# tum-vision/tandem

Hardware: AMD Instinct MI355X
Metric: depth-maps/sec @ 640×480×7-view×3-stage; TSDF voxels integrated/sec (higher is better)
Workload: dtype f32; 1 GPU; 640x480 ref+6-src keyframe window, 3-stage cascade (48/32/8 hypotheses), view aggregation, fp32; independent windows, 4 in flight per GPU (one DrMvsnet engine each) x 1 GPU replica(s); trained weights recovered from the reference's exported tandem_512x320 model (same architecture), inputs resident in HBM; height=480, width=640, views=7, parallelism=replicas x1, 4 engines per GPU

## Files before the change

### tandem_amd/csrc/conv_march.h

```cpp
#pragma once
#include "march_plan.h"

namespace dr {

struct MarchArgs {
  const int *tap2d;
  MarchGeom geo;
  int NPO;
  int ncols, colsH, colsW;
  int R, PS;
  int NP;
  int nit;
  int wsec;
  int NU;
  int steps;
  int ncw;
  int i_sv, i_sz, i_sy, o_sv, o_sz, o_sy;
  int depth;
  int inHp;
  int rm;
  int wino;
  int *err;
};

// ... 267 lines not shown
      s += sg.zb - sg.za;
    }
  }
}

template <int NRP, int CT, int PT>
struct MarchWSet {
  float4 g[3][CT], d[4][PT];
};
template <int NRP, int CT, int PT>
__device__ inline void march_w_load(const float4 *tile, const float4 *wsec, const int (&sw)[NRP][4][PT], int r, MarchWSet<NRP, CT, PT> &o) {
#pragma unroll
  for (int k = 0; k < 3; ++k)
#pragma unroll
    for (int ct = 0; ct < CT; ++ct) o.g[k][ct] = wsec[((r * 3 + k) * CT + ct) * 64];
#pragma unroll
  for (int pt = 0; pt < PT; ++pt)
#pragma unroll
    for (int q = 0; q < 4; ++q) o.d[q][pt] = tile[sw[r][q][pt]];
}
template <int NRP, int CT, int PT>
__device__ inline void march_w_anchor(const MarchWSet<NRP, CT, PT> &o) {
#pragma unroll
  for (int k = 0; k < 3; ++k)
#pragma unroll
    for (int ct = 0; ct < CT; ++ct) asm volatile("" ::"v"(o.g[k][ct].x), "v"(o.g[k][ct].y), "v"(o.g[k][ct].z), "v"(o.g[k][ct].w));
#pragma unroll
  for (int q = 0; q < 4; ++q)
#pragma unroll
    for (int pt = 0; pt < PT; ++pt) asm volatile("" ::"v"(o.d[q][pt].x), "v"(o.d[q][pt].y), "v"(o.d[q][pt].z), "v"(o.d[q][pt].w));
}
DR_HD inline float march_w_u1(float g0, float g1h, float g2) { return fmaf(g0 + g2, 0.5f, g1h); }
DR_HD inline float march_w_u2(float g0, float g1h, float g2) { return fmaf(g0 + g2, 0.5f, -g1h); }
template <int NRP, int CT, int PT>
__device__ inline void march_w_compute(MarchWSet<NRP, CT, PT> &o, floatx4 (&acc)[4][CT][PT]) {
  float4 u[4][CT];
#pragma unroll
  for (int ct = 0; ct < CT; ++ct) {
    const float4 g0 = o.g[0][ct], gh = o.g[1][ct], g2 = o.g[2][ct];
    u[0][ct] = g0; u[3][ct] = g2;
#ifdef DR_WABL_NO_WT
    u[1][ct] = gh; u[2][ct] = gh;
#else
    u[1][ct] = make_float4(march_w_u1(g0.x, gh.x, g2.x), march_w_u1(g0.y, gh.y, g2.y), march_w_u1(g0.z, gh.z, g2.z), march_w_u1(g0.w, gh.w, g2.w));
    u[2][ct] = make_float4(march_w_u2(g0.x, gh.x, g2.x), march_w_u2(g0.y, gh.y, g2.y), march_w_u2(g0.z, gh.z, g2.z), march_w_u2(g0.w, gh.w, g2.w));
#endif
  }
#ifndef DR_WABL_NO_IT
  conv_w_transform<PT>(o.d);
#endif
  conv_w_mfma<CT, PT>(u, o.d, acc);
}

template <int CT, int PT>
__device__ inline void march_epilogue_w(const ConvArgs &a, const MarchArgs &m, floatx4 (&acc)[4][CT][PT], const float4 (&scv)[CT], const float4 (&biv)[CT], int raw,
                                        int wave, int j, int g, int ct0, int zc, int z, int py0, int px0) {
#pragma unroll
  for (int pt = 0; pt < PT; ++pt) {
    const int tau = wave * PT + pt;
    const int xt = tau % a.TXT, yt = tau / a.TXT;
    const int qy = py0 + yt, qx = px0 + xt * 16 + j;
    if (qy >= a.nPH || qx >= a.nPW) continue;
#pragma unroll
    for (int ct = 0; ct < CT; ++ct) {
      const int c0 = (ct0 + ct) * 16 + 4 * g;
      if (c0 >= a.rows_valid) continue;
      const floatx4 m0 = acc[0][ct][pt], m1 = acc[1][ct][pt], m2 = acc[2][ct][pt], m3 = acc[3][ct][pt];
      const floatx4 o[2] = {(m0 + m1) + m2, (m1 - m2) - m3};
      size_t obase[2];
      float4 ps[2], ad[2];
#pragma unroll
      for (int r = 0; r < 2; ++r) {
        const int oy = 2 * qy + r;
        obase[r] = march_out_index(a, m, zc, z, oy, qx, c0);
        ps[r] = ad[r] = make_float4(0.f, 0.f, 0.f, 0.f);
        if (raw == 2) ps[r] = *reinterpret_cast<const float4 *>(a.out + obase[r]);
        if (raw != 1 && a.add_mode) {
          size_t abase = obase[r];
          if (a.add_mode == 2) abase = (((size_t)(zc + z) * a.addH + (oy >> 1)) * a.addW + (qx >> 1)) * a.outC + c0;
          ad[r] = *reinterpret_cast<const float4 *>(a.add + abase);
// ... 61 lines not shown
        asm volatile("" ::: "memory");
        const bool last = z == sg.zb - 1;
        auto tile_of = [&](int i) {
          int sl = cur.slot0 + lo + i;
          sl = sl >= R ? sl - R : sl;
          return (const float4 *)(lds4 + (size_t)sl * m.PS);
        };
        auto wsec_of = [&](int i) { return wp + (size_t)(lo + i) * m.wsec; };
        MarchWSet<NRP, CT, PT> set[2];
        march_w_load<NRP, CT, PT>(tile_of(0), wsec_of(0), sw, 0, set[0]);
#pragma unroll
        for (int i = 0; i < 3; ++i) {
          if (i < nsec) {
#pragma unroll
            for (int r = 0; r < NRP; ++r) {
              const int t = i * NRP + r;
              if (r + 1 < NRP) march_w_load<NRP, CT, PT>(tile_of(i), wsec_of(i), sw, r + 1, set[(t + 1) & 1]);
              else if (i + 1 < nsec) march_w_load<NRP, CT, PT>(tile_of(i + 1), wsec_of(i + 1), sw, 0, set[(t + 1) & 1]);
              __builtin_amdgcn_sched_barrier(0);
              march_w_compute<NRP, CT, PT>(set[t & 1], acc);
              __builtin_amdgcn_sched_barrier(0);
              if (r + 1 < NRP || i + 1 < nsec) march_w_anchor<NRP, CT, PT>(set[(t + 1) & 1]);
              if (r == NRP - 1 && (lo + i == 0 || last)) {
                asm volatile("" ::: "memory");
                if (lane == 0) flags[kMarchReleased + wave] = idx0 + lo + i + 1;
              }
            }
          }
        }
        march_epilogue_w<CT, PT>(a, m, acc, scv, biv, raw, wave, j, g, ct0, zc, z, py0, px0);
        cur.next_step(m.geo, R);
      }
      L += sg.nl;
      s += sg.zb - sg.za;
    }
  }
}

template <int CI>
__device__ inline void march_producer(const ConvArgs &a, const MarchArgs &m, float4 *lds4, march_flag_t *flags, float4 *wl, int pw, int lane, int s0,
                                      int s1, int NUP, int CT) {
  const int ct0 = blockIdx.z * CT, NS = m.geo.KZ * m.geo.NPI;
  int rel[kMarchMaxIt];
  unsigned yx[kMarchMaxIt];
#pragma unroll
  for (int it = 0; it < kMarchMaxIt; ++it) march_piece_entry<CI>(a, m, pw, it, lane, rel[it], yx[it]);
  const int depth = m.depth;
  int L = 0;
  for (int po = 0; po < m.NPO; ++po) {
    if (po > 0 && !march_wait_released(flags, m.ncw, L, m.err, lane)) return;
    for (int e = pw; e < NS * NUP * CT; e += kMarchProducers)
      conv_a_dma16(a.wpk + march_weight_src(a, m, po, e, NUP, CT, ct0) + lane, march_uniform(conv_a_lds_addr(wl + (size_t)e * 64)));
    int flight = 0;
    for (int s = s0; s < s1;) {
      const MarchSeg sg = march_segment(m.geo, s, s1);
      int zc, py0, px0;
      march_tile_origin(a, m, sg.col, zc, py0, px0);
      const int iy0 = m.rm ? 0 : py0 * a.sy - a.py, ix0 = px0 * a.sx - a.px;
      for (int l = 0; l < sg.nl; ++l) {
        const int idx = L + l;
        int plane, pi;
        march_load_plane(m.geo, sg, l, plane, pi);
#ifndef DR_MABL_FREE
        if (idx >= m.R && march_released_now(flags, m.ncw) < idx - m.R + 1) {
          if (flight) {
            conv_a_wait_dma();
// ... 93 lines not shown
          for (int c = 0; c < FZ / 4; ++c) { xi[4 * c] = xv[k][c].x; xi[4 * c + 1] = xv[k][c].y; xi[4 * c + 2] = xv[k][c].z; xi[4 * c + 3] = xv[k][c].w; }
#pragma unroll
          for (int sft = 0; sft < 4; ++sft)
#pragma unroll
            for (int gq = 0; gq < FZ / 4; ++gq)
#pragma unroll
              for (int r = 0; r < 4; ++r) acc4[r] = __builtin_fmaf(wr[r][4 * gq + sft], xi[4 * gq + sft], acc4[r]);
          float4 o = make_float4(0.f, 0.f, 0.f, 0.f);
          if (in[k]) { o.x = (acc4[0] + fb.x) + up[k].x; o.y = (acc4[1] + fb.y) + up[k].y; o.z = (acc4[2] + fb.z) + up[k].z; o.w = (acc4[3] + fb.w) + up[k].w; }
          if (pos < m.NP) dst[conv_a_unit<16>(pos, cg)] = o;
        }
      }
      asm volatile("" ::: "memory");
      if (lane == 0) flags[pw] = idx + 1;
    }
    L += sg.nl;
    s += sg.zb - sg.za;
  }
}

template <int CI, int NUP, int CT, int PT, int FZ = 0, int NCW = 8, int W = 0>
__global__ __launch_bounds__(64 * (NCW + (FZ ? kMarchFzProducers : kMarchProducers))) void k_conv_m(const ConvArgs a, const MarchArgs m) {
  extern __shared__ float4 lds4[];
  const int tid = threadIdx.x, lane = tid & 63, wave = march_uniform(tid >> 6);
  float4 *wl = lds4 + (size_t)m.R * m.PS;
  march_flag_t *flags = (march_flag_t *)(__attribute__((address_space(3))) char *)(wl + (size_t)m.geo.KZ * m.geo.NPI * m.wsec);
  if (tid < kMarchFlagInts) flags[tid] = 0;
  __syncthreads();
  const int nwg = gridDim.x, id = (int)(blockIdx.x & 7u) * (nwg >> 3) + (int)(blockIdx.x >> 3);
  int s0, s1;
  march_range(m.steps, id, nwg, s0, s1);
  if (s0 >= s1) return;
  if (wave < NCW) {
    if constexpr (W) march_consumer_w<CI, NUP, CT, PT, kMarchProducers>(a, m, lds4, flags, wl, wave, lane, s0, s1);
    else march_consumer<CI, NUP, CT, PT, (FZ ? kMarchFzProducers : kMarchProducers)>(a, m, lds4, flags, wl, wave, lane, s0, s1);
  }
  else if constexpr (FZ > 0) march_producer_fz<FZ>(a, m, lds4, flags, wl, wave - NCW, lane, s0, s1, NUP, CT);
  else march_producer<CI>(a, m, lds4, flags, wl, wave - NCW, lane, s0, s1, NUP, CT);
}

}
```

### tandem_amd/csrc/conv_mfma.h

```cpp
#pragma once
#include <algorithm>
#include <atomic>
#include <functional>

#include "dr_common.h"

namespace dr {

typedef float floatx4 __attribute__((ext_vector_type(4)));

struct ConvClass {
  int NU;
  int tap_base;
  int w_base;
  int ooz, ooy, oox;
};

struct ConvArgs {
  const float *in;
  float *out;
  const float4 *wpk;
  const float *scale, *bias, *add;
  const int *tapoff;
  const ConvClass *cls;
// ... 800 lines not shown
      ptrs.push_back(d);
      return d;
    }
    T *d = dalloc<T>(h.size());
    DR_HIP(hipMemcpy(d, h.data(), h.size() * sizeof(T), hipMemcpyHostToDevice));
    ptrs.push_back(d);
    return d;
  }
  ~DeviceArena() { for (void *p : ptrs) { if (host_only) free(p); else dfree(p); } }
};

struct ConvTuned {
  int Cin, Cout, kd, kh, kw, sd, sh, sw, transposed, mode, inD, inH, inW;
  int ci, ct, pt, tz, ty, txt;
  int async_;
};
#include "conv_tuned.h"

inline bool conv_instance_exists(int ci, int ct) {
  return (ci == 4 && ct == 1) || ((ci == 8 || ci == 16) && (ct == 1 || ct == 2 || ct == 4));
}
inline bool conv_a_instance_exists(int ci, int ct, int pt) {
  return (pt == 1 || pt == 2 || pt == 4) && ((ci == 4 && ct == 1 && pt != 1) || ((ci == 8 || ci == 16) && (ct == 1 || ct == 2)));
}
#define DR_MARCH_INSTANCES(X)                                                                                         \
  X(8, 6, 1, 2, 8) X(8, 6, 1, 4, 8) X(8, 6, 1, 1, 12) X(8, 6, 1, 2, 12)                                               \
  X(16, 12, 1, 2, 8) X(16, 12, 1, 4, 8) X(16, 12, 1, 1, 12) X(16, 12, 1, 2, 12)                                       \
  X(16, 9, 1, 2, 8) X(16, 9, 1, 4, 8) X(16, 9, 1, 1, 12) X(16, 9, 1, 2, 12) X(16, 9, 2, 2, 8)                         \
  X(8, 2, 1, 1, 8) X(8, 2, 1, 2, 8) X(8, 2, 1, 4, 8) X(8, 2, 1, 1, 10) X(8, 2, 1, 2, 10)                              \
  X(16, 4, 1, 1, 8) X(16, 4, 1, 2, 8) X(16, 4, 1, 4, 8) X(16, 4, 1, 1, 10) X(16, 4, 1, 2, 10)                         \
  X(16, 3, 1, 1, 8) X(16, 3, 1, 2, 8) X(16, 3, 1, 4, 8) X(16, 3, 1, 1, 10) X(16, 3, 1, 2, 10)                         \
  X(16, 3, 2, 1, 8) X(16, 3, 2, 2, 8) X(16, 3, 2, 1, 10) X(16, 3, 2, 2, 10)
#define DR_MARCH_W_INSTANCES(X) X(8, 6, 1, 1, 8) X(16, 12, 1, 1, 8) X(16, 9, 1, 1, 8)
inline bool conv_m_instance_exists(int ci, int nup, int ct, int pt, int ncw, bool wino = false) {
#define DR_X(CI_, NUP_, CT_, PT_, NCW_) if (ci == CI_ && nup == NUP_ && ct == CT_ && pt == PT_ && ncw == NCW_) return true;
  if (wino) { DR_MARCH_W_INSTANCES(DR_X) return false; }
  DR_MARCH_INSTANCES(DR_X)
#undef DR_X
  return false;
}
inline int conv_march_policy() {
  if (const char *e = getenv("DR_CONV_MARCH")) return atoi(e);
  return 1;
}
inline int conv_rowmarch_policy() {
  if (const char *e = getenv("DR_CONV_ROWMARCH")) return atoi(e);
  return 1;
}
struct MarchShape {
  int nup, npi, npo, ns, tyi, txi, np, ps, r, ncw;
  size_t wbytes, lds_bytes;
  long long steps;
  int grid;
  bool ok;
};
inline MarchShape march_shape(int KZ, int ntp, int Cin, int ci, int ct, int pt, int ty, int txt, int SX, int exy, int exx, int nPD, int nPH, int nPW, int CTtot,
                              bool rm = false, bool wino = false) {
  MarchShape m{};
  const int tpc = 16 / ci;
  if (Cin % ci || ntp % tpc || CTtot % ct || (ty * txt) % pt || (rm && (ty != 1 || KZ != 1)) || (wino && (KZ != 3 || rm || (ntp / 3) % tpc))) return m;
  m.ncw = ty * txt / pt;
  m.nup = ntp / tpc;
  if (!conv_m_instance_exists(ci, m.nup, ct, pt, m.ncw, wino)) return m;
  const int npass = Cin / ci, kz = rm ? 3 : KZ;
  if (npass > 2) return m;
  m.npi = KZ == 1 ? npass : 1; m.npo = KZ == 1 ? 1 : npass; m.ns = kz * m.npi;
// ... 165 lines not shown
      if (in_split && ci != in_split) continue;
      if (ci == 8 && L.Cin != 8) continue;
      for (int ncw : {8, 12})
      for (int pt : {1, 2, 4})
        for (int ty = 1; ty <= ncw * pt; ++ty) {
          if ((ncw * pt) % ty) continue;
          const int txt = ncw * pt / ty;
          if ((ty > 1 && ty / 2 >= nPH) || (txt > 1 && (txt / 2) * 16 >= nPW)) continue;
          for (int ct : {2, 1}) {
            const MarchShape ms = march_shape(L.kd, march_ntp, L.Cin, ci, ct, pt, ty, txt, SX, exy, exx, nPD, nPH, nPW, CTtot);
            if (!ms.ok || (fz && (ci != 16 || ct != 1 || ncw != 8))) continue;
            const double spw = std::ceil((double)ms.steps / ms.grid);
            const double unit = ms.ns * ms.nup * 4.0 * ct * pt * 32.0 * (ncw / 4) * (ncw == 12 ? 0.94 : 1.0);
            const double startup = (double)ms.lds_bytes / 16.0 + 3000.0;
            double cost = ms.npo * (spw * unit * 1.02 + startup);
            if (fz) cost *= 1.5;
            else if (L.kd == 1) cost *= 1.6;
            if (march_policy >= 2) cost *= 1e-3;
            cands.push_back({cost, ci, pt, ct, 1, ty, txt, L.kd, ms.tyi, ms.txi, 2});
          }
        }
    }
  }
  const int wino_policy_m = (!fz && !bf3) ? conv_wino_policy() : 0;
  if (march_ok && wino_policy_m >= 1 && L.kd == 3 && (R.outH & 1) == 0 && R.outH >= 2) {
    const int nPHw = R.outH / 2;
    for (int ci : {16, 8}) {
      if (in_split && ci != in_split) continue;
      if (ci == 8 && L.Cin != 8) continue;
      for (int ncw : {8})
        for (int ty = 1; ty <= ncw; ++ty) {
          if (ncw % ty) continue;
          const int txt = ncw / ty;
          if ((ty > 1 && ty / 2 >= nPHw) || (txt > 1 && (txt / 2) * 16 >= nPW)) continue;
          const MarchShape ms = march_shape(L.kd, march_ntp, L.Cin, ci, 1, 1, ty, txt, SX, exy, exx, nPD, nPHw, nPW, CTtot, false, true);
          if (!ms.ok) continue;
          const double spw = std::ceil((double)ms.steps / ms.grid);
          const double unit = ms.ns * (ms.nup / 3) * 16.0 * 32.0 * (ncw / 4) * (ncw == 12 ? 0.94 : 1.0);
          const double startup = (double)ms.lds_bytes / 16.0 + 3000.0;
          double cost = ms.npo * (spw * unit * 1.1 + startup);
          if (wino_policy_m >= 2) cost *= 1e-3 * 0.5;
          cands.push_back({cost, ci, 1, 1, 1, ty, txt, L.kd, ms.tyi, ms.txi, 5});
        }
    }
  }
  const bool rowmarch_ok = !fz && !bf3 && conv_rowmarch_policy() >= 1 && ncls == 1 && !L.transposed && !L.up2 && mode != CONV_X8 && L.kd == 1 && L.kh == 3 && L.kw == 3 &&
                           SZ == 1 && SY == 1 && L.sw == 1 && !add;
  const int row_ntp = rowmarch_ok ? (int)cx[0].t.size() : 0;
  if (rowmarch_ok) {
    for (int ci : {16, 8}) {
      if (in_split && ci != in_split) continue;
      if (ci == 8 && L.Cin != 8) continue;
      for (int ncw : {8, 10})
        for (int pt : {1, 2, 4}) {
          const int txt = ncw * pt;
          if (txt > 1 && (txt / 2) * 16 >= nPW) continue;
          for (int ct : {2, 1}) {
            const MarchShape ms = march_shape(L.kd, row_ntp, L.Cin, ci, ct, pt, 1, txt, SX, exy, exx, nPD, nPH, nPW, CTtot, true);
            if (!ms.ok) continue;
            const double spw = std::ceil((double)ms.steps / ms.grid);
            const double waste = (double)cdiv(nPW, txt * 16) * txt * 16 / nPW;
            const double unit = ms.ns * ms.nup * 4.0 * ct * pt * 32.0 * (ncw / 4.0) + 300.0;
            const double startup = (double)ms.lds_bytes / 16.0 + 3000.0;
            double cost = (spw * unit * 1.02 + startup) * 1.5;
            (void)waste;
            if (conv_rowmarch_policy() >= 2) cost *= 1e-3;
            cands.push_back({cost, ci, pt, ct, 1, 1, txt, 1, 1, ms.txi, 3});
// ... 273 lines not shown
    }
    const int ntiles = a.tilesD * a.tilesH * a.tilesW, split = CTtot / CT;
    const int wpc = cl.lds_bytes * 2 <= kConvMaxLds ? 2 : 1;
    const int want = std::max(1, std::min(ntiles, 256 * wpc / split));
    cl.grid = dim3(8 * cdiv(want, 8), 1, split);
  }
  if (ASYNC == 2 || ASYNC == 3 || ASYNC == 5) {
    const bool rm = ASYNC == 3;
    const MarchShape ms = rm ? march_shape(L.kd, row_ntp, L.Cin, CI, CT, PT, 1, TXT, SX, exy, exx, nPD, nPH, nPW, CTtot, true)
                             : march_shape(L.kd, march_ntp, L.Cin, CI, CT, PT, TY, TXT, SX, exy, exx, nPD, nPH, nPW, CTtot, false, wino_raw);
    if (!ms.ok) fail(DR_ERR_ARG, "plan_conv: inconsistent k_conv_m plan");
    cl.async = 2; cl.nup = ms.nup; cl.ncw = ms.ncw;
    a.zero16 = arena.upload(std::vector<float>(4, 0.f));
    a.a_slots = 0; a.a_wbufs = 0;
    MarchArgs &m = cl.march;
    const int kz = rm ? 3 : L.kd;
    std::vector<int> tap2d((size_t)ms.nup * TPC, 0);
    {
      const DimTaps &Y = *classes[0].y, &X = *classes[0].x;
      int n = 0;
      if (rm) for (size_t ix = 0; ix < X.t.size(); ++ix, ++n) tap2d[n] = X.off[ix];
      else for (size_t iy = 0; iy < Y.t.size(); ++iy) for (size_t ix = 0; ix < X.t.size(); ++ix, ++n) tap2d[n] = Y.off[iy] * TXI + X.off[ix];
    }
    m.tap2d = arena.upload(tap2d);
    m.geo.KZ = kz; m.geo.NPI = ms.npi; m.geo.Dc = rm ? nPH : (L.kd == 3 ? nPD : 1);
    m.NPO = ms.npo;
    m.colsH = rm ? 1 : cdiv(nPH, TY); m.colsW = cdiv(nPW, TXT * 16);
    m.ncols = (L.kd == 3 ? 1 : nPD) * m.colsH * m.colsW;
    m.R = ms.r; m.PS = ms.ps; m.NP = ms.np; m.nit = ms.ps / 128;
    m.wsec = ms.nup * CT * 64; m.NU = kz * ms.nup;
    m.steps = (int)ms.steps;
    m.ncw = ms.ncw;
    m.rm = rm ? 1 : 0;
    m.wino = wino_raw ? 1 : 0;
    const long long iplane = (long long)a.inH * a.inW * a.inC, oplane = (long long)a.outH * a.outW * a.outC;
    if (iplane * std::max(1, a.inD) >= (1ll << 31) || oplane * std::max(1, a.outD) >= (1ll << 31)) fail(DR_ERR_ARG, "plan_conv: tensor too large for k_conv_m's 32-bit strides");
    m.i_sv = L.kd == 3 ? 0 : (int)iplane; m.i_sz = rm ? a.inW * a.inC : (L.kd == 3 ? (int)iplane : 0); m.i_sy = rm ? 0 : a.inW * a.inC;
    m.o_sv = L.kd == 3 ? 0 : (int)oplane; m.o_sz = rm ? a.outW * a.outC : (L.kd == 3 ? (int)oplane : 0); m.o_sy = rm ? 0 : a.outW * a.outC;
    m.inHp = rm ? 1 : a.inH;
    m.err = arena.err_flag;
    m.depth = rm ? 3 : 2;
    if (const char *e = hook_env("DR_MARCH_PDEPTH")) m.depth = std::max(1, std::min(4, atoi(e)));
    cl.lds_bytes = ms.lds_bytes;
    cl.grid = dim3(ms.grid, 1, CTtot / CT);
  }
  cl.flops = flops;
  R.launches.push_back(cl);
  return R;
}

inline void conv_allow_big_lds(const void *fn, std::atomic<unsigned long long> &done, size_t lds_bytes) {
  if (lds_bytes <= 64 * 1024) return;
  int dev = 0;
  DR_HIP(hipGetDevice(&dev));
  const unsigned long long bit = 1ull << (dev & 63);
  if (done.load(std::memory_order_acquire) & bit) return;
  DR_HIP(hipFuncSetAttribute(fn, hipFuncAttributeMaxDynamicSharedMemorySize, (int)kConvMaxLds));
  done.fetch_or(bit, std::memory_order_release);
}
template <int CI, int CT, int PT, int FZ = 0>
inline void launch_conv_inst(const ConvLaunch &c, hipStream_t st) {
  static std::atomic<unsigned long long> done{0};
  conv_allow_big_lds(reinterpret_cast<const void *>(&k_conv<CI, CT, PT, FZ>), done, c.lds_bytes);
  hipLaunchKernelGGL((k_conv<CI, CT, PT, FZ>), c.grid, dim3(kConvThreads), c.lds_bytes, st, c.args);
}
#ifdef DR_PARITY_HOOKS
template <int CI, int CT, int PT>
// ... 28 lines not shown
  hipLaunchKernelGGL((k_conv_m<CI, NUP, CT, PT, FZ, NCW, W>), c.grid, dim3(64 * (NCW + (FZ ? kMarchFzProducers : kMarchProducers))), c.lds_bytes, st, c.args, c.march);
}
inline void launch_conv(const ConvLaunch &c, hipStream_t st) {
#ifndef DR_PARITY_HOOKS
  if (c.bf3) fail(DR_ERR_UNSUPPORTED, "launch_conv: the bf16 x 3 kernel is built with -DDR_PARITY_HOOKS only");
#else
  if (c.bf3) {
#define DR_CONV_B_CASE(CI_, CT_)                                                \
  if (c.ci == CI_ && c.ct == CT_ && !c.async && !c.fz) {                        \
    if (c.pt == 4) launch_conv_b_inst<CI_, CT_, 4>(c, st);                      \
    else launch_conv_b_inst<CI_, CT_, 1>(c, st);                                \
    return;                                                                     \
  }
    DR_CONV_B_CASE(8, 1)
    DR_CONV_B_CASE(8, 2)
    DR_CONV_B_CASE(8, 4)
    DR_CONV_B_CASE(16, 1)
    DR_CONV_B_CASE(16, 2)
    DR_CONV_B_CASE(16, 4)
#undef DR_CONV_B_CASE
    fail(DR_ERR_ARG, "launch_conv: no bf16x3 instance CI=%d CT=%d", c.ci, c.ct);
  }
#endif
#ifndef DR_PARITY_HOOKS
  if (c.fz) fail(DR_ERR_UNSUPPORTED, "launch_conv: fused-skip kernels are built with -DDR_PARITY_HOOKS only");
#else
  if (c.async == 2 && c.fz) {
    if (c.fz != 8 || c.ci != 16 || c.nup != 12 || c.ct != 1 || c.ncw != 8) fail(DR_ERR_ARG, "launch_conv: no fused-skip marching instance FZ=%d CI=%d NUP=%d CT=%d", c.fz, c.ci, c.nup, c.ct);
    if (c.pt == 4) launch_conv_m_inst<16, 12, 1, 4, 8>(c, st);
    else launch_conv_m_inst<16, 12, 1, 2, 8>(c, st);
    return;
  }
#endif
  if (c.async == 2 && c.march.wino) {
#define DR_X(CI_, NUP_, CT_, PT_, NCW_) \
  if (c.ci == CI_ && c.nup == NUP_ && c.ct == CT_ && c.pt == PT_ && c.ncw == NCW_) { launch_conv_m_inst<CI_, NUP_, CT_, PT_, 0, NCW_, 1>(c, st); return; }
    DR_MARCH_W_INSTANCES(DR_X)
#undef DR_X
    fail(DR_ERR_ARG, "launch_conv: no Winograd marching instance CI=%d NUP=%d CT=%d PT=%d waves=%d", c.ci, c.nup, c.ct, c.pt, c.ncw);
  }
  if (c.async == 2) {
#define DR_X(CI_, NUP_, CT_, PT_, NCW_) \
  if (c.ci == CI_ && c.nup == NUP_ && c.ct == CT_ && c.pt == PT_ && c.ncw == NCW_) { launch_conv_m_inst<CI_, NUP_, CT_, PT_, 0, NCW_>(c, st); return; }
    DR_MARCH_INSTANCES(DR_X)
#undef DR_X
    fail(DR_ERR_ARG, "launch_conv: no marching instance CI=%d NUP=%d CT=%d PT=%d waves=%d", c.ci, c.nup, c.ct, c.pt, c.ncw);
  }
  if (c.async == 4) {
#define DR_CONV_W_CASE(CI_, CT_, PT_) if (c.ci == CI_ && c.ct == CT_ && c.pt == PT_) { launch_conv_w_inst<CI_, CT_, PT_>(c, st); return; }
    DR_CONV_W_CASE(16, 1, 1) DR_CONV_W_CASE(16, 1, 2) DR_CONV_W_CASE(16, 2, 1) DR_CONV_W_CASE(16, 2, 2)
    DR_CONV_W_CASE(8, 1, 1) DR_CONV_W_CASE(8, 1, 2)
#undef DR_CONV_W_CASE
    fail(DR_ERR_ARG, "launch_conv: no Winograd instance CI=%d CT=%d PT=%d", c.ci, c.ct, c.pt);
  }
  if (c.async) {
#define DR_CONV_A_CASE(CI_, CT_)                                                \
  if (c.ci == CI_ && c.ct == CT_) {                                             \
    if (c.pt == 4) launch_conv_a_inst<CI_, CT_, 4>(c, st);                      \
    else if (c.pt == 2) launch_conv_a_inst<CI_, CT_, 2>(c, st);                 \
    else launch_conv_a_inst<CI_, CT_, 1>(c, st);                                \
    return;                                                                     \
  }
    if (c.ci == 4 && c.ct == 1 && c.pt == 1) fail(DR_ERR_ARG, "launch_conv: no async instance CI=4 PT=1");
    DR_CONV_A_CASE(4, 1)
    DR_CONV_A_CASE(8, 1)
    DR_CONV_A_CASE(8, 2)
    DR_CONV_A_CASE(16, 1)
    DR_CONV_A_CASE(16, 2)
#undef DR_CONV_A_CASE
    fail(DR_ERR_ARG, "launch_conv: no async instance CI=%d CT=%d PT=%d", c.ci, c.ct, c.pt);
  }
// ... 41 lines not shown
```

### tandem_amd/csrc/dr_mvsnet.hip

```cpp
#include <atomic>
#include <memory>

#include <dlfcn.h>
#include <rccl/rccl.h>

#include "conv_mfma.h"
#include "mvs_host.h"
#include "mvs_launch.h"
#ifdef DR_PARITY_HOOKS
#include "tail_kernels.h"
#endif
#include "fn_front.h"
#include "fn_head3.h"

namespace dr {

std::string &last_error_slot() {
  thread_local std::string s;
  return s;
}

struct DevTensor {
  float *d = nullptr;
  int D = 0, H = 0, W = 0, C = 0;
// ... 1274 lines not shown
    L.transposed = transposed == 1; L.weight = weight; L.relu = relu != 0;
    const bool up2 = transposed == 2;
    if (scale) L.scale.assign(scale, scale + Cout);
    if (bias) L.bias.assign(bias, bias + Cout);
    const ConvMode mode = (!transposed && sw == 1 && Cout == 8) ? CONV_XPAIR : ((!transposed && sw == 1 && Cout == 1) ? CONV_X8 : CONV_NORMAL);
    auto cz = axis_classes(kd, sd, L.transposed, D), cy = axis_classes(kh, sh, L.transposed, H), cx = axis_classes(kw, sw, L.transposed, W);
    const int oD = L.transposed ? D * sd : cz[0].npos, oH = L.transposed ? H * sh : (up2 ? 2 * H : cy[0].npos), oW = L.transposed ? W * sw : (up2 ? 2 * W : cx[0].npos);
    std::vector<float> hin(in, in + (size_t)D * H * W * Cin);
    float *d_in = arena.upload(hin);
    const size_t on = (size_t)oD * oH * oW * Cout;
    float poison; memcpy(&poison, &guard::kWord, 4);
    float *d_out = arena.upload(std::vector<float>(on, poison));
    float *d_add = nullptr;
    if (add) {
      const size_t an = add_up2 ? (size_t)oD * (oH / 2) * (oW / 2) * Cout : on;
      std::vector<float> ha(add, add + an);
      d_add = arena.upload(ha);
    }
    const char *rk = getenv("DR_CONV_RANK");
    ConvPlanOut P;
    for (int py = 0; py < (up2 ? 2 : 1); ++py) {
      L.up2 = up2 ? 1 + py : 0;
      P = plan_conv(L, mode, d_in, D, H, W, Cin, d_out, d_add, add_up2 ? 2 : 1, arena, rk ? atoi(rk) : 0);
      for (auto &cl : P.launches) launch_conv(cl, nullptr);
    }
    DR_HIP(hipDeviceSynchronize());
    DR_HIP(hipGetLastError());
    int march_err = 0;
    DR_HIP(hipMemcpy(&march_err, arena.err_flag, sizeof(int), hipMemcpyDeviceToHost));
    if (march_err) fail(DR_ERR_DEVICE, "k_conv_m: a ring wait gave up (code %d)", march_err);
    if (getenv("DR_CONV_PRINT")) {
      const ConvLaunch &c = P.launches.at(0);
      fprintf(stderr, "debug_conv: %s<%d,%d,%d> nup %d tile %dx%dx%d lds %zu grid %ux%u (%d candidates)%s\n", *conv_kind_name(c) ? conv_kind_name(c) : (c.bf3 ? "bf16x3" : "sync"), c.ci, c.ct, c.pt,
              c.nup, c.args.TZ, c.args.TY, c.args.TXT * 16, c.lds_bytes, c.grid.x, c.grid.z, P.ncand, c.args.class_loop ? ", class loop" : "");
    }
    DR_HIP(hipMemcpy(out, d_out, on * 4, hipMemcpyDeviceToHost));
    if (out_dims) { out_dims[0] = oD; out_dims[1] = oH; out_dims[2] = oW; }
  });
}

int drm_debug_tail(int device, const float *x, const float *skip, const float *w_deconv, const float *scale8, const float *bias8, const float *w_prob, int D, int h,
                   int w, int qy, int zchunk, int form, float *out) {
  return guarded([&] {
    using namespace dr;
#ifndef DR_PARITY_HOOKS
    fail(DR_ERR_UNSUPPORTED, "drm_debug_tail: k_tail / k_tail_m are built into the parity library (libdr_mi355x_hooks.so, -DDR_PARITY_HOOKS) only");
#else
    int n = 0;
    if (hipGetDeviceCount(&n) != hipSuccess || n <= device) fail(DR_ERR_DEVICE, "no HIP device %d", device);
    if (D <= 0 || h <= 0 || w <= 0 || (D | h | w) & 1) fail(DR_ERR_ARG, "drm_debug_tail: output dims must be positive and even");
    DR_HIP(hipSetDevice(device));
    DeviceArena arena;
    TailArgs t{};
    t.x = arena.upload(std::vector<float>(x, x + (size_t)(D / 2) * (h / 2) * (w / 2) * 16));
    t.skip = arena.upload(std::vector<float>(skip, skip + (size_t)D * h * w * 8));
    t.wd = arena.upload(tail_pack_deconv(w_deconv));
    std::vector<float> sb(scale8, scale8 + 8);
    sb.insert(sb.end(), bias8, bias8 + 8);
    t.sb = arena.upload(sb);
    t.wp = arena.upload(tail_pack_prob(w_prob));
    float poison; memcpy(&poison, &guard::kWord, 4);
    float *d_out = arena.upload(std::vector<float>((size_t)D * h * w, poison));
    t.out = d_out; t.D = D; t.h = h; t.w = w;
    const bool mf = form == 1;
    t.wmf = mf ? arena.upload(tail_pack_deconv_mfma(w_deconv)) : nullptr;
    tail_set_tile(t, qy, zchunk, mf);
    launch_tail(t, nullptr);
// ... 9 lines not shown
```

### tandem_amd/csrc/march_plan.h

```cpp
#pragma once
#if defined(__HIPCC__)
#define DR_HD __host__ __device__
#else
#define DR_HD
#endif

namespace dr {

struct MarchGeom {
  int Dc;
  int KZ;
  int NPI;
};
struct MarchSeg {
  int col, za, zb;
  int p0;
  int nl;
};

DR_HD inline MarchSeg march_segment(const MarchGeom &g, int s, int s1) {
  MarchSeg r;
  r.col = s / g.Dc;
  r.za = s - r.col * g.Dc;
  r.zb = r.za + (s1 - s) < g.Dc ? r.za + (s1 - s) : g.Dc;
// ... 2 lines not shown
    const int p1 = r.zb < g.Dc ? r.zb : g.Dc - 1;
    r.nl = (p1 - r.p0 + 1) * g.NPI;
  } else {
    r.p0 = r.za;
    r.nl = (r.zb - r.za) * g.NPI;
  }
  return r;
}
DR_HD inline int march_section_load(const MarchGeom &g, const MarchSeg &sg, int z, int sec) {
  const int dz = sec / g.NPI, pi = sec - dz * g.NPI;
  const int plane = g.KZ == 3 ? z - 1 + dz : z;
  if (plane < 0 || plane >= g.Dc) return -1;
  return (plane - sg.p0) * g.NPI + pi;
}
DR_HD inline bool march_section_releases(const MarchGeom &g, const MarchSeg &sg, int z, int sec) {
  return g.KZ == 1 || sec / g.NPI == 0 || z == sg.zb - 1;
}
DR_HD inline void march_load_plane(const MarchGeom &g, const MarchSeg &sg, int l, int &plane, int &pi) {
  plane = sg.p0 + l / g.NPI;
  pi = l % g.NPI;
}
struct MarchCursor {
  int rel0, slot0;
  DR_HD void begin(const MarchGeom &g, const MarchSeg &sg, int L, int R) {
    rel0 = (sg.za - (g.KZ == 3 ? 1 : 0) - sg.p0) * g.NPI;
    slot0 = (L + rel0 + 2 * R) % R;
  }
  DR_HD void next_step(const MarchGeom &g, int R) {
    rel0 += g.NPI;
    slot0 = slot0 + g.NPI >= R ? slot0 + g.NPI - R : slot0 + g.NPI;
  }
};

DR_HD inline void march_range(long long steps, int id, int n, int &s0, int &s1) {
  s0 = (int)(steps * id / n);
  s1 = (int)(steps * (id + 1) / n);
}

}
```

Before: 591.2 depth-maps/s.

## Add scatter-order Winograd marching consumer that reuses each input plane across three outputs

Adds a new Winograd marching-conv consumer that visits each loaded input depth plane once and scatters its contribution into three rotating output accumulators (one per kernel z-tap), instead of gathering three planes per output step. Each input tile is read and input-transformed once per plane rather than once per kz tap. The aim is to cut LDS traffic and repeated input transforms. In exchange it triples the accumulator register footprint, which risks register pressure and lower occupancy. It also changes ring release timing and makes this path the default, keeping the old gather order only behind an env var in parity builds.

```diff
diff --git a/tandem_amd/csrc/conv_march.h b/tandem_amd/csrc/conv_march.h
--- a/tandem_amd/csrc/conv_march.h
+++ b/tandem_amd/csrc/conv_march.h
@@ -323,12 +323,11 @@
 }
 DR_HD inline float march_w_u1(float g0, float g1h, float g2) { return fmaf(g0 + g2, 0.5f, g1h); }
 DR_HD inline float march_w_u2(float g0, float g1h, float g2) { return fmaf(g0 + g2, 0.5f, -g1h); }
-template <int NRP, int CT, int PT>
-__device__ inline void march_w_compute(MarchWSet<NRP, CT, PT> &o, floatx4 (&acc)[4][CT][PT]) {
-  float4 u[4][CT];
+template <int CT>
+__device__ inline void march_w_derive(const float4 (&g)[3][CT], float4 (&u)[4][CT]) {
 #pragma unroll
   for (int ct = 0; ct < CT; ++ct) {
-    const float4 g0 = o.g[0][ct], gh = o.g[1][ct], g2 = o.g[2][ct];
+    const float4 g0 = g[0][ct], gh = g[1][ct], g2 = g[2][ct];
     u[0][ct] = g0; u[3][ct] = g2;
 #ifdef DR_WABL_NO_WT
     u[1][ct] = gh; u[2][ct] = gh;
@@ -337,6 +336,11 @@
     u[2][ct] = make_float4(march_w_u2(g0.x, gh.x, g2.x), march_w_u2(g0.y, gh.y, g2.y), march_w_u2(g0.z, gh.z, g2.z), march_w_u2(g0.w, gh.w, g2.w));
 #endif
   }
+}
+template <int NRP, int CT, int PT>
+__device__ inline void march_w_compute(MarchWSet<NRP, CT, PT> &o, floatx4 (&acc)[4][CT][PT]) {
+  float4 u[4][CT];
+  march_w_derive<CT>(o.g, u);
 #ifndef DR_WABL_NO_IT
   conv_w_transform<PT>(o.d);
 #endif
@@ -464,6 +468,175 @@
         cur.next_step(m.geo, R);
       }
       L += sg.nl;
+      s += sg.zb - sg.za;
+    }
+  }
+}
+
+template <int CT>
+struct MarchSG { float4 g[3][CT]; };
+template <int PT>
+struct MarchSD { float4 d[4][PT]; };
+template <int K>
+struct MarchPath { static constexpr int value = K; };
+template <int CT>
+__device__ inline void march_s_load_g(const float4 *wsec, int r, MarchSG<CT> &o) {
+#pragma unroll
+  for (int k = 0; k < 3; ++k)
+#pragma unroll
+    for (int ct = 0; ct < CT; ++ct) o.g[k][ct] = wsec[((r * 3 + k) * CT + ct) * 64];
+}
+template <int NRP, int PT>
+__device__ inline void march_s_load_d(const float4 *tile, const unsigned (&sw)[NRP][2][PT], int r, MarchSD<PT> &o) {
+  const char *tb = reinterpret_cast<const char *>(tile);
+#pragma unroll
+  for (int pt = 0; pt < PT; ++pt)
+#pragma unroll
+    for (int h = 0; h < 2; ++h) {
+      const unsigned x = sw[r][h][pt];
+      o.d[2 * h][pt] = *reinterpret_cast<const float4 *>(tb + (x & 0xffffu));
+      o.d[2 * h + 1][pt] = *reinterpret_cast<const float4 *>(tb + (x >> 16));
+    }
+}
+template <int CT>
+__device__ inline void march_s_anchor_g(const MarchSG<CT> &o) {
+#pragma unroll
+  for (int k = 0; k < 3; ++k)
+#pragma unroll
+    for (int ct = 0; ct < CT; ++ct) asm volatile("" ::"v"(o.g[k][ct].x), "v"(o.g[k][ct].y), "v"(o.g[k][ct].z), "v"(o.g[k][ct].w));
+}
+template <int PT>
+__device__ inline void march_s_anchor_d(const MarchSD<PT> &o) {
+#pragma unroll
+  for (int q = 0; q < 4; ++q)
+#pragma unroll
+    for (int pt = 0; pt < PT; ++pt) asm volatile("" ::"v"(o.d[q][pt].x), "v"(o.d[q][pt].y), "v"(o.d[q][pt].z), "v"(o.d[q][pt].w));
+}
+
+template <int CI, int NUP, int CT, int PT, int NPW>
+__device__ inline void march_consumer_ws(const ConvArgs &a, const MarchArgs &m, float4 *lds4, march_flag_t *flags, const float4 *wl, int wave, int lane,
+                                         int s0, int s1) {
+  static_assert(NUP % 3 == 0 && NUP >= 6, "three kernel rows per chunk of x taps, at least two chunks per plane");
+  constexpr int TPC = 16 / CI, NRP = NUP / 3, NG = 3 * NRP;
+  constexpr int WSEC = NUP * CT * 64;
+  const int j = lane & 15, g = lane >> 4;
+  const int sub = (4 * g) / CI, c4 = ((4 * g) % CI) / 4, ct0 = blockIdx.z * CT;
+  unsigned sw[NRP][2][PT];
+#pragma unroll
+  for (int pt = 0; pt < PT; ++pt) {
+    const int bpos = march_bpos(a, wave, pt, PT, j);
+#pragma unroll
+    for (int r = 0; r < NRP; ++r)
+#pragma unroll
+      for (int h = 0; h < 2; ++h) {
+        const unsigned lo = 16u * (unsigned)conv_a_unit<CI>(bpos + m.tap2d[r * TPC + sub] + (2 * h) * a.TXI, c4);
+        const unsigned hi = 16u * (unsigned)conv_a_unit<CI>(bpos + m.tap2d[r * TPC + sub] + (2 * h + 1) * a.TXI, c4);
+        sw[r][h][pt] = lo | (hi << 16);
+        asm volatile("" : "+v"(sw[r][h][pt]));
+      }
+  }
+  const float4 *wp = wl + lane;
+  const int R = m.R, Dc = m.geo.Dc;
+  floatx4 acc[3][4][CT][PT];
+  auto clear = [&](floatx4 (&s)[4][CT][PT]) {
+#pragma unroll
+    for (int p = 0; p < 4; ++p)
+#pragma unroll
+      for (int ct = 0; ct < CT; ++ct)
+#pragma unroll
+        for (int pt = 0; pt < PT; ++pt) s[p][ct][pt] = floatx4{0.f, 0.f, 0.f, 0.f};
+  };
+  auto move = [&](floatx4 (&d)[4][CT][PT], const floatx4 (&s)[4][CT][PT]) {
+#pragma unroll
+    for (int p = 0; p < 4; ++p)
+#pragma unroll
+      for (int ct = 0; ct < CT; ++ct)
+#pragma unroll
+        for (int pt = 0; pt < PT; ++pt) {
+          d[p][ct][pt] = s[p][ct][pt];
+        }
+  };
+  clear(acc[0]); clear(acc[1]); clear(acc[2]);
+  MarchSD<PT> dd[2];
+  MarchSG<CT> gg[2];
+  int cached = 0, idx = 0, slot = 0;
+  for (int po = 0; po < m.NPO; ++po) {
+    const int raw = m.NPO == 1 ? 0 : (po == 0 ? 1 : 2);
+    for (int s = s0; s < s1;) {
+      const MarchSeg sg = march_segment(m.geo, s, s1);
+      int zc, py0, px0;
+      march_tile_origin(a, m, sg.col, zc, py0, px0);
+      for (int i = 0; i < sg.nl; ++i) {
+        const int p = sg.p0 + i;
+        const bool more = i + 1 < sg.nl || s + (sg.zb - sg.za) < s1;
+        const bool on[3] = {march_plane_feeds(sg, p, 0), march_plane_feeds(sg, p, 1), march_plane_feeds(sg, p, 2)};
+        const float4 *tile = lds4 + (size_t)slot * m.PS;
+        auto plane = [&](auto main_path) -> bool {
+          constexpr bool MAIN = decltype(main_path)::value != 0;
+          if (!march_wait_ready<NPW>(flags, idx, cached, m.err, lane)) return false;
+          asm volatile("" ::: "memory");
+          march_s_load_g<CT>(wp, 0, gg[0]);
+          march_s_load_d<NRP, PT>(tile, sw, 0, dd[0]);
+#pragma unroll
+          for (int r = 0; r < NRP; ++r) {
+#pragma unroll
+            for (int dz = 0; dz < 3; ++dz) {
+              const int t = r * 3 + dz;
+              MarchSG<CT> &gn = gg[(t + 1) & 1];
+              MarchSD<PT> &dn = dd[(r + 1) & 1];
+              if (t + 1 < NG) {
+                march_s_load_g<CT>(wp + (size_t)((dz + 1) % 3) * WSEC, dz == 2 ? r + 1 : r, gn);
+                if (dz == 2) march_s_load_d<NRP, PT>(tile, sw, r + 1, dn);
+              }
+              __builtin_amdgcn_sched_barrier(0);
+              if (dz == 0) conv_w_transform<PT>(dd[r & 1].d);
+              if (MAIN || on[dz]) {
+                float4 u[4][CT];
+                march_w_derive<CT>(gg[t & 1].g, u);
+                conv_w_mfma<CT, PT>(u, dd[r & 1].d, acc[2 - dz]);
+              }
+              __builtin_amdgcn_sched_barrier(0);
+              if (t + 1 < NG) {
+                march_s_anchor_g<CT>(gn);
+                if (dz == 2) march_s_anchor_d<PT>(dn);
+              }
+              if ((MAIN || more) ? (r == NRP - 2 && dz == 2) : t == NG - 2) {
+                asm volatile("" ::: "memory");
+                if (lane == 0) flags[kMarchReleased + wave] = idx + 1;
+              }
+            }
+          }
+          const float *scp = a.scale, *bip = a.bias;
+          int el = lane;
+          asm volatile("" : "+s"(scp), "+s"(bip), "+v"(el));
+          const int j = el & 15, g = el >> 4;
+          float4 scv[CT], biv[CT];
+          if (MAIN || on[2] || on[1]) {
+#pragma unroll
+            for (int ct = 0; ct < CT; ++ct) {
+              scv[ct] = *reinterpret_cast<const float4 *>(scp + (ct0 + ct) * 16 + 4 * g);
+              biv[ct] = *reinterpret_cast<const float4 *>(bip + (ct0 + ct) * 16 + 4 * g);
+            }
+          }
+          if (MAIN || on[2]) {
+            march_epilogue_w<CT, PT>(a, m, acc[0], scv, biv, raw, wave, j, g, ct0, zc, p - 1, py0, px0);
+          }
+          if (!MAIN && on[1] && p == Dc - 1) {
+            march_epilogue_w<CT, PT>(a, m, acc[1], scv, biv, raw, wave, j, g, ct0, zc, p, py0, px0);
+            clear(acc[1]);
+          }
+          __builtin_amdgcn_sched_barrier(0);
+          move(acc[0], acc[1]);
+          move(acc[1], acc[2]);
+          clear(acc[2]);
+          __builtin_amdgcn_sched_barrier(0);
+          return true;
+        };
+        const bool inner = more && on[0] && on[1] && on[2];
+        if (!(inner ? plane(MarchPath<1>{}) : plane(MarchPath<0>{}))) return;
+        ++idx;
+        slot = slot + 1 == R ? 0 : slot + 1;
+      }
       s += sg.zb - sg.za;
     }
   }
@@ -623,7 +796,8 @@
   march_range(m.steps, id, nwg, s0, s1);
   if (s0 >= s1) return;
   if (wave < NCW) {
-    if constexpr (W) march_consumer_w<CI, NUP, CT, PT, kMarchProducers>(a, m, lds4, flags, wl, wave, lane, s0, s1);
+    if constexpr (W == 2) march_consumer_ws<CI, NUP, CT, PT, kMarchProducers>(a, m, lds4, flags, wl, wave, lane, s0, s1);
+    else if constexpr (W) march_consumer_w<CI, NUP, CT, PT, kMarchProducers>(a, m, lds4, flags, wl, wave, lane, s0, s1);
     else march_consumer<CI, NUP, CT, PT, (FZ ? kMarchFzProducers : kMarchProducers)>(a, m, lds4, flags, wl, wave, lane, s0, s1);
   }
   else if constexpr (FZ > 0) march_producer_fz<FZ>(a, m, lds4, flags, wl, wave - NCW, lane, s0, s1, NUP, CT);
diff --git a/tandem_amd/csrc/conv_mfma.h b/tandem_amd/csrc/conv_mfma.h
--- a/tandem_amd/csrc/conv_mfma.h
+++ b/tandem_amd/csrc/conv_mfma.h
@@ -856,6 +856,11 @@
   X(16, 3, 1, 1, 8) X(16, 3, 1, 2, 8) X(16, 3, 1, 4, 8) X(16, 3, 1, 1, 10) X(16, 3, 1, 2, 10)                         \
   X(16, 3, 2, 1, 8) X(16, 3, 2, 2, 8) X(16, 3, 2, 1, 10) X(16, 3, 2, 2, 10)
 #define DR_MARCH_W_INSTANCES(X) X(8, 6, 1, 1, 8) X(16, 12, 1, 1, 8) X(16, 9, 1, 1, 8)
+inline int conv_march_w_order(int ci, int nup) {
+  (void)ci; (void)nup;
+  if (const char *e = hook_env("DR_MARCH_W_ORDER")) return atoi(e) == 1 ? 1 : 2;
+  return 2;
+}
 inline bool conv_m_instance_exists(int ci, int nup, int ct, int pt, int ncw, bool wino = false) {
 #define DR_X(CI_, NUP_, CT_, PT_, NCW_) if (ci == CI_ && nup == NUP_ && ct == CT_ && pt == PT_ && ncw == NCW_) return true;
   if (wino) { DR_MARCH_W_INSTANCES(DR_X) return false; }
@@ -1087,7 +1092,7 @@
         for (int ty = 1; ty <= ncw; ++ty) {
           if (ncw % ty) continue;
           const int txt = ncw / ty;
-          if ((ty > 1 && ty / 2 >= nPHw) || (txt > 1 && (txt / 2) * 16 >= nPW)) continue;
+          if (!hook_env("DR_MARCH_ANY_TILE") && ((ty > 1 && ty / 2 >= nPHw) || (txt > 1 && (txt / 2) * 16 >= nPW))) continue;
           const MarchShape ms = march_shape(L.kd, march_ntp, L.Cin, ci, 1, 1, ty, txt, SX, exy, exx, nPD, nPHw, nPW, CTtot, false, true);
           if (!ms.ok) continue;
           const double spw = std::ceil((double)ms.steps / ms.grid);
@@ -1427,7 +1432,7 @@
     m.steps = (int)ms.steps;
     m.ncw = ms.ncw;
     m.rm = rm ? 1 : 0;
-    m.wino = wino_raw ? 1 : 0;
+    m.wino = wino_raw ? conv_march_w_order(CI, ms.nup) : 0;
     const long long iplane = (long long)a.inH * a.inW * a.inC, oplane = (long long)a.outH * a.outW * a.outC;
     if (iplane * std::max(1, a.inD) >= (1ll << 31) || oplane * std::max(1, a.outD) >= (1ll << 31)) fail(DR_ERR_ARG, "plan_conv: tensor too large for k_conv_m's 32-bit strides");
     m.i_sv = L.kd == 3 ? 0 : (int)iplane; m.i_sz = rm ? a.inW * a.inC : (L.kd == 3 ? (int)iplane : 0); m.i_sy = rm ? 0 : a.inW * a.inC;
@@ -1522,11 +1527,21 @@
     return;
   }
 #endif
+  if (c.async == 2 && c.march.wino == 2) {
+#define DR_X(CI_, NUP_, CT_, PT_, NCW_) \
+  if (c.ci == CI_ && c.nup == NUP_ && c.ct == CT_ && c.pt == PT_ && c.ncw == NCW_) { launch_conv_m_inst<CI_, NUP_, CT_, PT_, 0, NCW_, 2>(c, st); return; }
+    DR_MARCH_W_INSTANCES(DR_X)
+#undef DR_X
+  }
+#ifdef DR_PARITY_HOOKS
   if (c.async == 2 && c.march.wino) {
 #define DR_X(CI_, NUP_, CT_, PT_, NCW_) \
   if (c.ci == CI_ && c.nup == NUP_ && c.ct == CT_ && c.pt == PT_ && c.ncw == NCW_) { launch_conv_m_inst<CI_, NUP_, CT_, PT_, 0, NCW_, 1>(c, st); return; }
     DR_MARCH_W_INSTANCES(DR_X)
 #undef DR_X
+  }
+#endif
+  if (c.async == 2 && c.march.wino) {
     fail(DR_ERR_ARG, "launch_conv: no Winograd marching instance CI=%d NUP=%d CT=%d PT=%d waves=%d", c.ci, c.nup, c.ct, c.pt, c.ncw);
   }
   if (c.async == 2) {
diff --git a/tandem_amd/csrc/dr_mvsnet.hip b/tandem_amd/csrc/dr_mvsnet.hip
--- a/tandem_amd/csrc/dr_mvsnet.hip
+++ b/tandem_amd/csrc/dr_mvsnet.hip
@@ -1330,7 +1330,8 @@
     if (getenv("DR_CONV_PRINT")) {
       const ConvLaunch &c = P.launches.at(0);
       fprintf(stderr, "debug_conv: %s<%d,%d,%d> nup %d tile %dx%dx%d lds %zu grid %ux%u (%d candidates)%s\n", *conv_kind_name(c) ? conv_kind_name(c) : (c.bf3 ? "bf16x3" : "sync"), c.ci, c.ct, c.pt,
-              c.nup, c.args.TZ, c.args.TY, c.args.TXT * 16, c.lds_bytes, c.grid.x, c.grid.z, P.ncand, c.args.class_loop ? ", class loop" : "");
+              c.nup, c.args.TZ, c.args.TY, c.args.TXT * 16, c.lds_bytes, c.grid.x, c.grid.z, P.ncand,
+              c.args.class_loop ? ", class loop" : (c.async == 2 && c.march.wino ? (c.march.wino == 2 ? ", scatter order" : ", gather order") : ""));
     }
     DR_HIP(hipMemcpy(out, d_out, on * 4, hipMemcpyDeviceToHost));
     if (out_dims) { out_dims[0] = oD; out_dims[1] = oH; out_dims[2] = oW; }
diff --git a/tandem_amd/csrc/march_plan.h b/tandem_amd/csrc/march_plan.h
--- a/tandem_amd/csrc/march_plan.h
+++ b/tandem_amd/csrc/march_plan.h
@@ -58,6 +58,15 @@
   }
 };
 
+DR_HD inline bool march_plane_feeds(const MarchSeg &sg, int p, int dz) {
+  const int zo = p + 1 - dz;
+  return zo >= sg.za && zo < sg.zb;
+}
+DR_HD inline void march_plane_completes(const MarchGeom &g, const MarchSeg &sg, int p, int &lo, int &hi) {
+  lo = p - 1 >= sg.za ? p - 1 : p;
+  hi = (p == g.Dc - 1 && p < sg.zb) ? p + 1 : p;
+}
+
 DR_HD inline void march_range(long long steps, int id, int n, int &s0, int &s1) {
   s0 = (int)(steps * id / n);
   s1 = (int)(steps * (id + 1) / n);
```

Result: faster. 599.3 depth-maps/s, median of 6 (+1.4%).
